# marcinmiklitz/pywindow

Hardware: AMD Instinct MI355X
Metric: trajectory frames/sec full_analysis (pore+windows), CC3 1k-frame (higher is better)
Workload: dtype f64

## Files before the change

pywindow_amd/csrc/pw_kernels.hip:

```cpp
#include <hip/hip_runtime.h>
#include <atomic>
#include <stdio.h>
#include <stdlib.h>
#include <string.h>
#include <time.h>

#include <algorithm>
#include <mutex>
#include <new>

#include "../../include/pywindow_amd.h"
#include "pw_host.hpp"
#include "pw_stat_host.hpp"
#include <vector>
#include "pw_unit.hpp"
#include "pw_launch.hpp"

using namespace pw;

extern "C" int pw_hostpath_run(const pw_batch_in* in, unsigned stages, pw_unit_out* out, const pw_params* prm, int p_cap,
                               int threads, pw_unit_debug* dbg, pw_extra_window* xw, unsigned xw_cap, unsigned* xw_count);
extern "C" int pw_hostpath_default_threads(void);
extern "C" void pw_hostpath_math(int which, const double* x, const double* y, long n, double* out);
extern "C" size_t pw_internal_big_block_bytes(int nmax, int p_cap);
// ... 456 lines not shown
    HostBatch* host;
    long n_units;
    long n_atoms;
    int nmax;
    int vstride;
    unsigned long long* d_ready;
    unsigned long long* h_ready;
    long ready_units;
    int pending;
    unsigned pending_stages;
    long* d_offset;
    double* d_xyz;
    double* d_vdw;
    double* d_mass;
    unsigned char* d_tmpl;
    void* block;
    size_t block_bytes;
    void* parts[5];
    size_t part_bytes[5];
    pw_unit_out* d_out;
    pw_unit_out* d_outs[PW_SETS];
    pw_extra_window* d_xw[PW_SETS];
    unsigned* d_xw_count;
    unsigned xw_cap;
    int nbuf;
    int cur;
    hipEvent_t ev_read[PW_SETS];
    int read_valid[PW_SETS];
    int written_set[PW_SETS];
};

static int block_take(pw_context* c, size_t bytes, void** out, size_t* got) {
    bytes = (bytes + 65535) & ~(size_t)65535;
    int best = -1;
    for (int i = 0; i < (int)c->blocks->size(); ++i) {
        const size_t b = (*c->blocks)[i].bytes;
        if (b >= bytes && b <= 2 * bytes + (1u << 20) && (best < 0 || b < (*c->blocks)[best].bytes)) best = i;
    }
    if (best >= 0) {
        *out = (*c->blocks)[best].p;
        *got = (*c->blocks)[best].bytes;
        c->blocks_bytes -= *got;
        c->blocks->erase(c->blocks->begin() + best);
        return PW_OK;
    }
    HIP_TRY(hipMalloc(out, bytes));
    *got = bytes;
    return PW_OK;
}
static void block_give(pw_context* c, void* p, size_t bytes) {
    if (!p) return;
    if (c && c->blocks && c->blocks->size() < 96 && c->blocks_bytes + bytes <= ((size_t)8 << 30)) {
        c->blocks->push_back({p, bytes});
// ... 98 lines not shown
    if (getenv("PW_PLAN_DEBUG"))
        fprintf(stderr, "launch NW=%d mask %x grid %d lds %zu nmax %d units %ld atoms %ld\n", NW, MASK, p.grid, p.lds,
                r->nmax, r->n_units, r->n_atoms);
    {
        static std::atomic<unsigned long long> done{0};
        unsigned long long bit = 1ull << (c->device & 63);
        if (!(done.load(std::memory_order_acquire) & bit)) {
            HIP_TRY(hipFuncSetAttribute((const void*)kern, hipFuncAttributeMaxDynamicSharedMemorySize,
                                        160 * 1024 - 256 - (int)PW_KERNEL_STATIC_LDS));
            done.fetch_or(bit, std::memory_order_release);
        }
    }
    if (reset_counter) HIP_TRY(hipMemsetAsync(c->counter + counter_slot, 0, sizeof(unsigned long long), st));
    PwWsArgs wsa;
    wsa.ws = c->ws + ws_first;
    wsa.slab = c->slab + (size_t)ws_first * team_slab_bytes(c->p_cap);
    wsa.adj = adj_first >= 0 ? c->adj + (size_t)adj_first * team_adj_words(c->p_cap) : (unsigned long long*)nullptr;
    wsa.xwin = r->d_xw[r->cur];
    wsa.xwin_count = r->d_xw_count + r->cur;
    wsa.xwin_cap = r->xw_cap;
    wsa.p_cap = c->p_cap;
    wsa.nb_off = c->nb_off; wsa.nb_idx = c->nb_idx; wsa.nb_bound = c->nb_bound; wsa.nb_unit = c->nb_unit;
    wsa.wait_ticks = c->wait_ticks * (1 + r->nmax / 512); wsa.stream_wait_ticks = c->stream_wait_ticks;
    hipLaunchKernelGGL(kern, dim3(p.grid), dim3(NW * 64), p.lds, st, r->n_units, r->d_offset,
                       r->d_xyz, r->d_vdw, r->d_mass, stages, r->nmax, p.nrot, p.nlb, p.nframes, p.lean, wsa,
                       c->counter + counter_slot, r->d_out, role, c->cur_queue, c->cur_slots, c->prm, c->rsq_tab,
                       r->vstride, (const unsigned long long*)r->d_ready, (const unsigned char*)r->d_tmpl);
    HIP_TRY(hipGetLastError());
    return PW_OK;
}
static int launch_plan(pw_context* c, pw_resident* r, unsigned stages, const LaunchPlan& p, hipStream_t st,
                       int ws_first, int adj_first, int counter_slot, int role = PW_ROLE_PLAIN,
                       bool reset_counter = true) {
    if (stages == MASK_CHAINS && p.nw == 1)
        return launch_nw<1, MASK_CHAINS>(c, r, stages, p, st, ws_first, adj_first, counter_slot, role, reset_counter);
    if (stages == MASK_WINDOWS && p.nw == 4)
        return launch_nw<4, MASK_WINDOWS>(c, r, stages, p, st, ws_first, adj_first, counter_slot, role, reset_counter);
    if (stages == MASK_WINDOWS_AVG && p.nw == 4)
        return launch_nw<4, MASK_WINDOWS_AVG>(c, r, stages, p, st, ws_first, adj_first, counter_slot, role, reset_counter);
    if (p.nw == 1 && (stages & ~MASK_CHAINS) == 0)
        return launch_nw<1, MASK_CHAINS>(c, r, stages, p, st, ws_first, adj_first, counter_slot, role, reset_counter);
    if (p.nw != 4) {
        snprintf(g_err, sizeof(g_err), "internal: no kernel for %d-wave teams with stages 0x%x", p.nw, stages);
        return PW_E_BAD_ARG;
    }
    return launch_nw<4, MASK_ANY>(c, r, stages, p, st, ws_first, adj_first, counter_slot, role, reset_counter);
// ... 451 lines not shown
                HIP_TRY(hipDeviceSynchronize());
                if (c->bigmem) HIP_TRY(hipFree(c->bigmem));
                c->bigmem = nullptr;
                c->bigmem_bytes = 0;
                HIP_TRY(hipMalloc((void**)&c->bigmem, bb * (size_t)grid));
                c->bigmem_bytes = bb * (size_t)grid;
            }
            c->need_fork = 1;
            rc = join_pipeline(c);
            if (rc != PW_OK) return rc;
            if (r->read_valid[r->cur]) {
                HIP_TRY(hipStreamWaitEvent(c->stream, r->ev_read[r->cur], 0));
                r->read_valid[r->cur] = 0;
            }
            r->written_set[r->cur] = -1;
            HIP_TRY(hipMemsetAsync(r->d_xw_count + r->cur, 0, sizeof(unsigned), c->stream));
            HIP_TRY(hipMemsetAsync(c->counter + 4 * PW_SETS + 1, 0, sizeof(unsigned long long), c->stream));
            PwWsArgs wsa;
            wsa.ws = c->ws; wsa.slab = c->slab; wsa.adj = c->adj;
            wsa.xwin = r->d_xw[r->cur]; wsa.xwin_count = r->d_xw_count + r->cur; wsa.xwin_cap = r->xw_cap;
            wsa.p_cap = c->p_cap;
            wsa.nb_off = c->nb_off; wsa.nb_idx = c->nb_idx; wsa.nb_bound = c->nb_bound; wsa.nb_unit = c->nb_unit;
            wsa.wait_ticks = c->wait_ticks; wsa.stream_wait_ticks = c->stream_wait_ticks;
            return pw_internal_big_launch((void*)c->stream, (int)grid, r->n_units, r->d_offset, r->d_xyz, r->d_vdw, r->d_mass,
                                          stages, r->nmax, &wsa, c->bigmem, bb, c->counter + 4 * PW_SETS + 1, r->d_out, &c->prm,
                                          c->rsq_tab, r->vstride);
        }
    }
    const bool large = wanted_p_cap(c) > PW_P_CAP_PIPELINE;
    const bool pipeline = !c->fused && (stages & PW_STAGE_WINDOWS) != 0 && !large;
    if (!pipeline) {
        LaunchPlan p;
        bool win = (stages & PW_STAGE_WINDOWS) != 0;
        bool opt = win || (stages & PW_STAGE_OPT);
        rc = plan_launch(c, r->n_units, r->nmax, (win || (stages & PW_STAGE_AVG)) ? 4 : 1, win,
                         win ? -1 : (opt ? 1 : 0), &p);
        if (rc != PW_OK) return rc;
        if (large) {
            const size_t per = team_ws_bytes(wanted_p_cap(c), win);
            const size_t budget = (size_t)48 << 30;
            if (per > ((size_t)192 << 30)) {
                snprintf(g_err, sizeof(g_err), "%d sampling vectors per molecule need %zu GB of workspace per team",
                         wanted_p_cap(c), per >> 30);
                return PW_E_TOO_LARGE;
            }
            long g = (long)(budget / per);
// ... 216 lines not shown
            if (n <= 0) snprintf(g_err, sizeof(g_err), "unit %ld has %ld atoms", u, n);
            else snprintf(g_err, sizeof(g_err), "unit %ld has %ld atoms, the template %ld", u, n, (long)in->template_atoms);
            return PW_E_BAD_ARG;
        }
        if (n > nmax) nmax = (int)n;
    }
    r->nmax = nmax;
    r->vstride = in->template_atoms > 0 ? 0 : 1;
    const long nconst = in->template_atoms > 0 ? (long)in->template_atoms : natoms;
#define UP_TRY(call)                          \
    do {                                      \
        hipError_t e_ = (call);               \
        if (e_ != hipSuccess) {               \
            set_err(#call, e_);               \
            pw_resident_free(c, r);           \
            return PW_E_HIP;                  \
        }                                     \
    } while (0)
    if (r->n_units) {
        r->nbuf = c->nsets ? c->nsets : auto_sets(r->n_units);
        auto up256 = [](size_t b) { return (b + 255) & ~(size_t)255; };
        const size_t b_off = up256(sizeof(long) * (size_t)(r->n_units + 1)), b_xyz = up256(sizeof(double) * 3 * (size_t)natoms);
        const size_t b_con = up256(sizeof(double) * (size_t)nconst);
        const size_t b_out = up256((size_t)r->nbuf * sizeof(pw_unit_out) * (size_t)r->n_units + 64);
        const size_t b_tmpl = in->template_atoms > 0 ? up256(template_groups_bytes(nmax)) : 0;
        {
            int rcb = block_take(c, b_off + b_xyz + 2 * b_con + b_tmpl + b_out, &r->block, &r->block_bytes);
            if (rcb != PW_OK) { pw_resident_free(c, r); return rcb; }
        }
        unsigned char* base = (unsigned char*)r->block;
        r->d_offset = (long*)base; base += b_off;
        r->d_xyz = (double*)base; base += b_xyz;
        r->d_vdw = (double*)base; base += b_con;
        r->d_mass = (double*)base; base += b_con;
        std::vector<unsigned char> tmpl_host;
        if (b_tmpl) {
            r->d_tmpl = base; base += b_tmpl;
            tmpl_host.resize(template_groups_bytes(nmax));
            template_groups_build(in->vdw, in->mass, nmax, tmpl_host.data());
        }
        r->d_outs[0] = (pw_unit_out*)base;
        for (int k = 1; k < r->nbuf; ++k) r->d_outs[k] = r->d_outs[0] + (size_t)k * r->n_units;
        r->d_xw_count = (unsigned*)(r->d_outs[0] + (size_t)r->nbuf * r->n_units);
        for (int k = 0; k < PW_SETS; ++k) r->written_set[k] = -1;
        r->d_out = r->d_outs[0];
        r->cur = 0;
        UP_TRY(hipMemcpyAsync(r->d_offset, in->atom_offset, sizeof(long) * (r->n_units + 1),
                              hipMemcpyHostToDevice, c->stream));
        UP_TRY(hipMemcpyAsync(r->d_xyz, in->xyz, sizeof(double) * 3 * natoms, hipMemcpyHostToDevice,
                              c->stream));
        UP_TRY(hipMemcpyAsync(r->d_vdw, in->vdw, sizeof(double) * nconst, hipMemcpyHostToDevice,
                              c->stream));
        UP_TRY(hipMemcpyAsync(r->d_mass, in->mass, sizeof(double) * nconst, hipMemcpyHostToDevice,
                              c->stream));
        if (r->d_tmpl) UP_TRY(hipMemcpyAsync(r->d_tmpl, tmpl_host.data(), tmpl_host.size(), hipMemcpyHostToDevice, c->stream));
        UP_TRY(hipMemsetAsync(r->d_outs[0], 0, r->nbuf * sizeof(pw_unit_out) * r->n_units + 64, c->stream));
        UP_TRY(hipStreamSynchronize(c->stream));
    }
#undef UP_TRY
    c->need_fork = 1;
    *out = r;
    return PW_OK;
}

int pw_resident_stream_begin(pw_context* c, int64_t n_units, int64_t template_atoms, const double* vdw, const double* mass,
                             pw_resident** out) {
    if (!c || !out || n_units <= 0 || template_atoms <= 0 || !vdw || !mass) return PW_E_BAD_ARG;
    PW_LOCK_CONTEXT(c);
    *out = nullptr;
    PW_HOST_UNSUPPORTED(c, "streamed batches");
    if (template_atoms > 40000 || n_units * template_atoms > (int64_t)1 << 40) return PW_E_TOO_LARGE;
    {
        const int pcap = wanted_p_cap(c) > c->p_cap ? wanted_p_cap(c) : c->p_cap;
        if (UnitShared::bytes((int)template_atoms, 1, 1, 1, false, pcap) + 64 > 160 * 1024 - 256 - PW_KERNEL_STATIC_LDS) {
            snprintf(g_err, sizeof(g_err), "molecule with %ld atoms: beyond LDS, upload it in one piece", (long)template_atoms);
            return PW_E_TOO_LARGE;
        }
    }
    PW_ON_DEVICE(c->device);
    pw_resident* r = new (std::nothrow) pw_resident();
    if (!r) return PW_E_NOMEM;
    memset((void*)r, 0, sizeof(*r));
    r->n_units = (long)n_units;
    r->n_atoms = (long)(n_units * template_atoms);
    r->nmax = (int)template_atoms;
    r->vstride = 0;
    r->nbuf = c->nsets ? c->nsets : auto_sets(r->n_units);
    auto up256 = [](size_t b) { return (b + 255) & ~(size_t)255; };
    const size_t b_off = up256(sizeof(long) * (size_t)(r->n_units + 1)), b_xyz = up256(sizeof(double) * 3 * (size_t)r->n_atoms);
    const size_t b_con = up256(sizeof(double) * (size_t)template_atoms);
    const size_t b_out = up256((size_t)r->nbuf * sizeof(pw_unit_out) * (size_t)r->n_units + 64);
    const size_t b_tmpl = up256(template_groups_bytes((int)template_atoms));
    int rcb = block_take(c, b_off + b_xyz + 2 * b_con + b_tmpl + b_out + 256, &r->block, &r->block_bytes);
    if (rcb != PW_OK) { pw_resident_free(c, r); return rcb; }
    unsigned char* base = (unsigned char*)r->block;
    r->d_offset = (long*)base; base += b_off;
    r->d_xyz = (double*)base; base += b_xyz;
    r->d_vdw = (double*)base; base += b_con;
    r->d_mass = (double*)base; base += b_con;
    r->d_tmpl = base; base += b_tmpl;
    std::vector<unsigned char> tmpl_host(template_groups_bytes((int)template_atoms));
    template_groups_build(vdw, mass, (int)template_atoms, tmpl_host.data());
    r->d_outs[0] = (pw_unit_out*)base; base += b_out;
    {
        constexpr unsigned RING = 4096;
        if (!c->ready_vals) {
            hipError_t eh = hipHostMalloc((void**)&c->ready_vals, RING * sizeof(unsigned long long), hipHostMallocMapped | hipHostMallocCoherent);
            if (eh == hipSuccess) eh = hipHostGetDevicePointer((void**)&c->ready_dev, c->ready_vals, 0);
            if (eh != hipSuccess) { set_err("pw_resident_stream_begin (ready counters)", eh); c->ready_vals = nullptr; pw_resident_free(c, r); return PW_E_HIP; }
        }
        const unsigned at = c->ready_at++ % RING;
        r->h_ready = c->ready_vals + at;
        r->d_ready = c->ready_dev + at;
        __atomic_store_n(r->h_ready, 0ull, __ATOMIC_RELEASE);
    }
    for (int k = 1; k < r->nbuf; ++k) r->d_outs[k] = r->d_outs[0] + (size_t)k * r->n_units;
    r->d_xw_count = (unsigned*)(r->d_outs[0] + (size_t)r->nbuf * r->n_units);
    for (int k = 0; k < PW_SETS; ++k) r->written_set[k] = -1;
    r->d_out = r->d_outs[0];
    std::vector<long> off((size_t)r->n_units + 1);
    for (long u = 0; u <= r->n_units; ++u) off[(size_t)u] = u * (long)template_atoms;
    hipError_t e = hipMemcpyAsync(r->d_offset, off.data(), sizeof(long) * (r->n_units + 1), hipMemcpyHostToDevice, c->stream);
    if (e == hipSuccess) e = hipMemcpyAsync(r->d_vdw, vdw, sizeof(double) * template_atoms, hipMemcpyHostToDevice, c->stream);
    if (e == hipSuccess) e = hipMemcpyAsync(r->d_mass, mass, sizeof(double) * template_atoms, hipMemcpyHostToDevice, c->stream);
    if (e == hipSuccess) e = hipMemcpyAsync(r->d_tmpl, tmpl_host.data(), tmpl_host.size(), hipMemcpyHostToDevice, c->stream);
    if (e == hipSuccess) e = hipMemsetAsync(r->d_outs[0], 0, r->nbuf * sizeof(pw_unit_out) * r->n_units + 64, c->stream);
    if (e == hipSuccess) e = hipStreamSynchronize(c->stream);
    if (e != hipSuccess) { set_err("pw_resident_stream_begin", e); pw_resident_free(c, r); return PW_E_HIP; }
    c->need_fork = 1;
    *out = r;
    return PW_OK;
}

int pw_resident_stream_append(pw_context* c, pw_resident* r, const double* xyz, int64_t first, int64_t count) {
    if (!c || !r || !xyz || count < 0) return PW_E_BAD_ARG;
    PW_LOCK_CONTEXT(c);
    if (!r->d_ready || first != r->ready_units || first + count > r->n_units) {
        snprintf(g_err, sizeof(g_err), "pw_resident_stream_append: units %ld..%ld do not continue the %ld appended so far (of %ld)",
                 (long)first, (long)(first + count), r->ready_units, r->n_units);
        return PW_E_BAD_ARG;
    }
    if (count == 0) return PW_OK;
    PW_ON_DEVICE(c->device);
    const size_t per = (size_t)r->nmax * 3;
    HIP_TRY(hipMemcpyAsync(r->d_xyz + (size_t)first * per, xyz, sizeof(double) * per * (size_t)count, hipMemcpyHostToDevice, c->stream));
    HIP_TRY(hipStreamSynchronize(c->stream));
    r->ready_units = (long)(first + count);
    __atomic_store_n(r->h_ready, (unsigned long long)r->ready_units, __ATOMIC_RELEASE);
    if (r->pending && r->ready_units == r->n_units) return pw_resident_launch(c, r, r->pending_stages);
    return PW_OK;
}

int pw_internal_resident_adopt(pw_context* c, long n_units, long n_atoms, int nmax, long* d_offset, double* d_xyz,
                               double* d_vdw, double* d_mass, const size_t* part_bytes, pw_resident** out) {
    if (!c || !out || n_units <= 0 || nmax <= 0 || !part_bytes) return PW_E_BAD_ARG;
    PW_LOCK_CONTEXT(c);
    PW_HOST_UNSUPPORTED(c, "device batches");
    PW_ON_DEVICE(c->device);
    pw_resident* r = new (std::nothrow) pw_resident();
    if (!r) return PW_E_NOMEM;
    memset((void*)r, 0, sizeof(*r));
    r->nbuf = c->nsets ? c->nsets : auto_sets(n_units);
    void* outs = nullptr;
    size_t outs_bytes = 0;
    int rcb = block_take(c, r->nbuf * sizeof(pw_unit_out) * (size_t)n_units + 64, &outs, &outs_bytes);
    if (rcb != PW_OK) { delete r; return rcb; }
    r->d_outs[0] = (pw_unit_out*)outs;
    hipError_t e = hipMemsetAsync(r->d_outs[0], 0, r->nbuf * sizeof(pw_unit_out) * n_units + 64, c->stream);
    if (e == hipSuccess) e = hipStreamSynchronize(c->stream);
    if (e != hipSuccess) {
        set_err("pw_internal_resident_adopt", e);
        block_give(c, outs, outs_bytes);
        delete r;
        return PW_E_HIP;
    }
    r->n_units = n_units; r->n_atoms = n_atoms; r->nmax = nmax; r->vstride = 1;
    r->d_offset = d_offset; r->d_xyz = d_xyz; r->d_vdw = d_vdw; r->d_mass = d_mass;
    r->parts[0] = d_offset; r->parts[1] = d_xyz; r->parts[2] = d_vdw; r->parts[3] = d_mass; r->parts[4] = outs;
    for (int k = 0; k < 4; ++k) r->part_bytes[k] = part_bytes[k];
    r->part_bytes[4] = outs_bytes;
    for (int k = 1; k < r->nbuf; ++k) r->d_outs[k] = r->d_outs[0] + (size_t)k * n_units;
    r->d_xw_count = (unsigned*)(r->d_outs[0] + (size_t)r->nbuf * n_units);
    for (int k = 0; k < PW_SETS; ++k) r->written_set[k] = -1;
    r->d_out = r->d_outs[0];
    r->cur = 0;
    c->need_fork = 1;
    *out = r;
    return PW_OK;
}

static int fetch_extra_windows(pw_context* c, pw_resident* r, unsigned count) {
    c->extra->clear();
    if (count == 0) return PW_OK;
    if (count > r->xw_cap) {
        HIP_TRY(hipDeviceSynchronize());
        if (r->d_xw[0]) HIP_TRY(hipFree(r->d_xw[0]));
        for (int k = 0; k < PW_SETS; ++k) r->d_xw[k] = nullptr;
        r->xw_cap = 0;
        const unsigned cap = ((count + count / 2 + 1023u) / 1024u) * 1024u;
        HIP_TRY(hipMalloc((void**)&r->d_xw[0], (size_t)r->nbuf * cap * sizeof(pw_extra_window)));
        for (int k = 1; k < r->nbuf; ++k) r->d_xw[k] = r->d_xw[0] + (size_t)k * cap;
        r->xw_cap = cap;
        snprintf(g_err, sizeof(g_err), "%u windows beyond the %d a record holds: launch the analysis again "
                 "(the list for them has been allocated)", count, PW_W_MAX);
        return PW_E_RETRY;
// ... 511 lines not shown
```

pywindow_amd/csrc/pw_launch.hpp:

```cpp
#pragma once
#include "../../include/pywindow_amd.h"

struct PwWsArgs {
    void* ws;
    unsigned char* slab;
    unsigned long long* adj;
    pw_extra_window* xwin;
    unsigned* xwin_count;
    unsigned xwin_cap;
    int p_cap;
    const unsigned* nb_off;
    const unsigned short* nb_idx;
    const double* nb_bound;
    const double* nb_unit;
    long long wait_ticks;
    long long stream_wait_ticks;
};

struct UnitQueue {
    unsigned long long tail;
    unsigned long long head;
    int error;
    int started;
};
enum : int { PW_ROLE_PLAIN = 0, PW_ROLE_PRODUCER = 1, PW_ROLE_CONSUMER = 2 };

#if defined(__HIPCC__)
template <class WS>
__device__ inline void bind_workspace(WS* ws, const PwWsArgs& a, unsigned team, const unsigned* rsq_tab, size_t slab_bytes,
                                      size_t adj_words) {
    bind_team_slab(ws, a.slab + (size_t)team * slab_bytes, a.p_cap);
    ws->adj = a.adj ? a.adj + (size_t)team * adj_words : nullptr;
    ws->xwin = a.xwin; ws->xwin_count = a.xwin_count; ws->xwin_cap = a.xwin_cap;
    ws->nb_off = a.nb_off; ws->nb_idx = a.nb_idx; ws->nb_bound = a.nb_bound; ws->nb_unit = a.nb_unit;
    ws->rsq = rsq_tab;
}
#endif
```

pywindow_amd/csrc/pw_unit.hpp:

```cpp
#pragma once
#include "../../include/pywindow_amd.h"
#include "pw_lbfgsb.hpp"
#include "pw_math.hpp"
#include "pw_team.hpp"
#include <string.h>

#if defined(PW_PROFILE) && defined(__HIPCC__)
__shared__ unsigned long long pw_prof_lds[32];
#define PW_PROF_BASE(ws) ((unsigned long long*)pw_prof_lds)
#endif
#if defined(PW_PROFILE) && defined(__HIP_DEVICE_COMPILE__)
#define PW_T0(var) long long var = wall_clock64()
#if defined(PW_ZPROF) && defined(PW_LB_FINE)
#define PW_T1(ws, slot, var) do { (void)var; } while (0)
#elif defined(PW_BARRIER_PROF)
#define PW_T1(ws, slot, var) do { (void)var; if (T::lane() == 0) { unsigned long long w_ = 0; \
        for (int k_ = 0; k_ < T::NWAVES; ++k_) w_ += atomicExch(&pw_bar_acc[k_], 0ull); \
        atomicAdd(&pw_prof_lds[slot], w_); } } while (0)
#else
#define PW_T1(ws, slot, var) do { if (T::lane() == 0) atomicAdd(&pw_prof_lds[slot], (unsigned long long)(wall_clock64() - var)); } while (0)
#endif
#else
#define PW_T0(var) do {} while (0)
#define PW_T1(ws, slot, var) do {} while (0)
// ... 29 lines not shown
    double* pts;
    double* vals;
    int* surv_k;
    int* labels;
    unsigned char* flag;
    unsigned long long* adj;
    double* xw;
    int* xw_ok;
    int p_cap;
    const unsigned* nb_off;
    const unsigned short* nb_idx;
    const double* nb_unit;
    const double* nb_bound;
    pw_extra_window* xwin;
    unsigned* xwin_count;
    unsigned xwin_cap;
    double leaf[256];
    double acc8[8 * 160];
    int leaf_tab[324];
    unsigned long long prof[32];
    const unsigned* rsq;
    pw_unit_debug* dbg_base;
    long unit;
};
PW_HD inline size_t team_slab_bytes(int p_cap) { return (size_t)p_cap * 192; }
PW_HD inline size_t team_adj_words(int p_cap) { return (size_t)p_cap * (size_t)(p_cap / 64); }
PW_HD inline int round_p_cap(long p) {
    if (p < PW_P_MAX) p = PW_P_MAX;
    return (int)((p + 127) & ~127l);
}
PW_HD inline int params_p_cap(double adjust_windows, double adjust_average) {
    double a = adjust_windows > adjust_average ? adjust_windows : adjust_average;
    if (!(a > 0.0)) a = 1.0;
    double want = 2100.0 * a;
    if (want > 4.0e6) want = 4.0e6;
    return round_p_cap((long)want + 1);
}
PW_HD inline void bind_team_slab(TeamWorkspace* ws, unsigned char* slab, int p_cap) {
    const size_t p = (size_t)p_cap;
    double* d = (double*)slab;
    ws->knn = d; d += 10 * p;
    ws->pts = d; d += 3 * p;
    ws->vals = d; d += p;
    ws->xw = d; d += 7 * p;
    int* i = (int*)d;
    ws->surv_k = i; i += p;
// ... 9 lines not shown
    int mw_given;
    double centroid[3];
    double maxd;
    int maxd_i, maxd_j;
    double pore_g;
    int pore_atom;
    double opt_c[3];
    double opt_g;
    int opt_atom;
    double shift[3];
    ClassInfo cls;
    int cls_cnt[PW_KCLS];
    double eps;
    double radius;
    int P;
    int n_surv;
    int n_clusters;
    int n_eval;
    int status;
    double red_v[16];
    int red_i[16];
    int md_list[64];
    int md_count;
    int win_first;
    double win_vec[PW_W_MAX][3];
    int win_ok[PW_W_MAX];
    double win_d[PW_W_MAX];
    double win_c[PW_W_MAX][3];
};

struct UnitShared {
    PW_LDS UnitVars* v;
    ldouble* vdw;
    ldouble* mass;
    lint* perm;
    lint* inv;
    Frame A;
    Frame S;
    Frame R[8];
    PW_LDS void* lb[8];
    PW_LDS unsigned long long* bits[3];
    size_t rot_words;
    int nslots;
    PW_LDS unsigned char* scratch;
    size_t scratch_bytes;
    PW_HD static size_t bytes(int nmax, int nrot, int nlb, int nframes = 2, int lean = 0, int pcap = PW_P_MAX) {
// ... 1682 lines not shown
    }
    PW_HD explicit GramEdgeRule(int n) {
        t0 = applies(n) ? 8 * (n / 8) : 0x40000000;
        panel = last_panel_start(n);
        panel_wide = 12 * (panel / 12);
        nfull = 32 * (n / 32);
        limlast = 12 * ((n - nfull) / 12);
    }
    PW_HD bool is_edge(int o) const { return (unsigned)(o - t0) < 4u; }
    PW_HD bool in_wide_kernel(int o) const {
        return o < panel ? o < panel_wide : (o & 31) < (o < nfull ? 24 : limlast);
    }
    PW_HD bool pair_uses_edge_order(int oi, int oj) const {
        return (is_edge(oi) && in_wide_kernel(oj)) || (is_edge(oj) && in_wide_kernel(oi));
    }
};
template <bool EDGE>
PW_HD inline __attribute__((always_inline)) double pw_gram_nn(double xi, double yi, double zi, double xj, double yj,
                                                              double zj, int oi, int oj, const GramEdgeRule& er) {
    if (EDGE && er.pair_uses_edge_order(oi, oj)) return pw_fma(zi, zj, xi * xj + yi * yj);
    return pw_fma(zi, zj, pw_fma(yi, yj, xi * xj));
}

#if defined(__HIP_DEVICE_COMPILE__)
template <class T, bool VALUE_ONLY, bool EDGE>
__device__ inline __attribute__((always_inline)) bool team_max_dim_few(UnitShared& sh, const Frame& F, int n,
                                                                       const GramEdgeRule& er, const double* centre) {
    auto& v = *sh.v;
    const double cx = centre ? centre[0] : 0.0, cy = centre ? centre[1] : 0.0, cz = centre ? centre[2] : 0.0;
    double smax = -PW_INF, nmax = 0.0;
    int imax = 0x7fffffff;
    for (int i = T::tid(); i < n; i += T::SIZE) {
        const double dx = F.x[i] - cx, dy = F.y[i] - cy, dz = F.z[i] - cz;
        const double si = pw_sqrt(dx * dx + dy * dy + dz * dz) + F.vdw[i];
        if (si > smax) { smax = si; imax = i; }
        nmax = pw_max(nmax, F.xx[i]);
    }
    T::wave_argmax(smax, imax);
    nmax = -T::wave_min(-nmax);
    if (T::lane() == 0) { v.red_v[T::wave()] = smax; v.red_i[T::wave()] = imax; v.red_v[8 + T::wave()] = nmax; }
    T::sync();
    {
        double bb = v.red_v[0], nn = v.red_v[8];
        int bi = v.red_i[0];
        for (int w = 1; w < T::NWAVES; ++w) {
            if (v.red_v[w] > bb || (v.red_v[w] == bb && v.red_i[w] < bi)) { bb = v.red_v[w]; bi = v.red_i[w]; }
            nn = pw_max(nn, v.red_v[8 + w]);
        }
        smax = bb; imax = bi; nmax = nn;
    }
// ... 1 lines not shown
    if (!(smax < PW_INF) || imax >= n) return false;
    const double xi = F.x[imax], yi = F.y[imax], zi = F.z[imax], xxi = F.xx[imax], vi = F.vdw[imax];
    const int oi = F.perm[imax];
    double L = -PW_INF;
    for (int j = T::tid(); j < n; j += T::SIZE) {
        const int oj = F.perm[j];
        double d = 0.0;
        if (j != imax) {
            const double gg = pw_gram_nn<EDGE>(xi, yi, zi, F.x[j], F.y[j], F.z[j], oi, oj, er);
            const double d2 = (oi < oj) ? pw_m2add(gg, xxi) + F.xx[j] : pw_m2add(gg, F.xx[j]) + xxi;
            d = pw_sqrt(d2 > 0.0 ? d2 : 0.0);
        }
        L = pw_max(L, d + (vi + F.vdw[j]));
    }
    L = -T::wave_min(-L);
    if (T::lane() == 0) v.red_v[T::wave()] = L;
    T::sync();
    L = v.red_v[0];
    for (int w = 1; w < T::NWAVES; ++w) L = pw_max(L, v.red_v[w]);
    T::sync();
    if (!(L < PW_INF)) return false;
    const double margin = 1e-6 + 4e-15 * nmax / pw_max(L, 1e-3);
    const double thr = (L - smax) - margin;
    if (T::tid() == 0) v.md_count = 0;
    T::sync();
    for (int i0 = 0; i0 < n; i0 += T::SIZE) {
        const int i = i0 + T::tid();
        bool in = false;
        if (i < n) {
            const double dx = F.x[i] - cx, dy = F.y[i] - cy, dz = F.z[i] - cz;
            in = pw_sqrt(dx * dx + dy * dy + dz * dz) + F.vdw[i] >= thr;
        }
        const unsigned long long mk = T::ballot(in);
        int base = 0;
        if (T::lane() == 0 && mk) base = atomicAdd((PW_LDS int*)&v.md_count, (int)__builtin_popcountll(mk));
        base = __builtin_amdgcn_readfirstlane(base);
        const int at = base + (int)__builtin_popcountll(mk & ((1ull << T::lane()) - 1ull));
        if (in && at < 64) v.md_list[at] = i;
    }
    T::sync();
    const int m = v.md_count;
    if (m > 64) { T::sync(); return false; }
    double bv = -PW_INF, bidx = PW_INF;
    for (int p = T::tid(); p < m * m; p += T::SIZE) {
        const int a = p / m, b = p - a * m;
        const int ia = v.md_list[a], ib = v.md_list[b];
        const int oa = F.perm[ia], ob = F.perm[ib];
        if (oa > ob) continue;
        double d = 0.0;
        if (ia != ib) {
            const double gg = pw_gram_nn<EDGE>(F.x[ia], F.y[ia], F.z[ia], F.x[ib], F.y[ib], F.z[ib], oa, ob, er);
            const double d2 = pw_m2add(gg, F.xx[ia]) + F.xx[ib];
            d = pw_sqrt(d2 > 0.0 ? d2 : 0.0);
        }
        const double val = d + (F.vdw[ia] + F.vdw[ib]);
        const double idx = (double)(oa * n + ob);
        if (val > bv || (val == bv && idx < bidx)) { bv = val; bidx = idx; }
    }
    int ii = (int)(bidx < 2147483647.0 ? bidx : 2147483647.0);
    T::wave_argmax(bv, ii);
    if (T::lane() == 0) { v.red_v[T::wave()] = bv; v.red_i[T::wave()] = ii; }
    T::sync();
    if (T::tid() == 0) {
        double bb = v.red_v[0];
        int bi = v.red_i[0];
        for (int w = 1; w < T::NWAVES; ++w) {
            const double vv = v.red_v[w];
            const int vi2 = v.red_i[w];
            if (vv > bb || (vv == bb && vi2 < bi)) { bb = vv; bi = vi2; }
        }
        v.maxd = bb;
        if (!VALUE_ONLY) { v.maxd_i = bi / n; v.maxd_j = bi % n; }
    }
    T::sync();
    return true;
}
#endif

template <class T, bool VALUE_ONLY = false, bool EDGE = false>
PW_HD inline __attribute__((always_inline)) void team_max_dim_body(UnitShared& sh, const Frame& F, int n,
                                                                   double* item_best = nullptr, const double* centre = nullptr) {
    const GramEdgeRule er(n);
#if defined(__HIP_DEVICE_COMPILE__)
    if (T::WSIZE == 64 && team_max_dim_few<T, VALUE_ONLY, EDGE>(sh, F, n, er, centre)) return;
#else
    (void)centre;
#endif
    const auto& C = *F.cls;
    const int ngrp = C.k;
    const int R = (n + 1) / 2;
    int K = 1;
    {
        long best_cost = 0x7fffffffffffffffl;
        for (int k = 1; k <= 4; ++k) {
            long passes = ((long)R * k + T::SIZE - 1) / T::SIZE;
            long cost = passes * ((n - 1 + 64 / k + k - 1) / k);
            if (cost < best_cost) { best_cost = cost; K = k; }
        }
    }
    const int nitem = R * K;
    double best = -PW_INF;
    if (ngrp > 0) {
        for (int t = T::tid(); t < nitem; t += T::SIZE) {
            const int p = t / K, q = t - p * K;
            double ibest = -PW_INF;
            for (int side = 0; side < 2; ++side) {
                const int i = side == 0 ? p : n - 1 - p;
                if (side == 1 && i == p) break;
                const double xi = F.x[i], yi = F.y[i], zi = F.z[i], xxi = F.xx[i], vi = F.vdw[i];
                const int oi = F.perm[i];
// ... 141 lines not shown
        for (int w = 1; w < T::NWAVES; ++w) bi = pw_min(bi, sh.v->red_v[w]);
        int idx = (int)bi;
        sh.v->maxd = vmax;
        sh.v->maxd_i = idx / n;
        sh.v->maxd_j = idx % n;
    }
    T::sync();
}

template <class T, bool VALUE_ONLY = false>
PW_HD inline __attribute__((always_inline)) void team_max_dim_impl(UnitShared& sh, const Frame& F, int n,
                                                                   double* item_best = nullptr, const double* centre = nullptr) {
    if (GramEdgeRule::applies(n)) team_max_dim_body<T, VALUE_ONLY, true>(sh, F, n, item_best, centre);
    else team_max_dim_body<T, VALUE_ONLY, false>(sh, F, n, item_best, centre);
}

template <class T, bool VALUE_ONLY = false>
PW_NOINLINE PW_HD inline void team_max_dim(UnitShared& sh, const Frame& F, int n, double* item_best = nullptr,
                                           const double* centre = nullptr) {
    team_max_dim_impl<T, VALUE_ONLY>(sh, F, n, item_best, centre);
}

template <class T>
PW_HD inline __attribute__((always_inline)) void stage_basic_impl(UnitShared& sh, TeamWorkspace* ws, int n,
                                                                  pw_unit_out* out, bool com_only) {
    auto& v = *sh.v;
    (void)ws;
    ldouble* cols = seq_sum_columns<T>(sh, n);
    if (cols) {
        const size_t np = (size_t)((n + 1) & ~1);
        for (int i = T::tid(); i < n; i += T::SIZE) {
            const int pos = sh.inv[i];
            const double m = sh.mass[i];
            cols[i] = sh.A.x[pos] * m; cols[np + i] = sh.A.y[pos] * m; cols[2 * np + i] = sh.A.z[pos] * m;
        }
    }
    if (T::tid() == 0 && !v.mw_given) v.mw = molecular_weight_sum((const double*)sh.mass, n);
    T::sync();
    if (cols) {
        seq_sum_columns_add<T>(cols, n, [&](int c, double s) { v.com[c] = s / v.mw; });
    } else {
    auto com_comp = [&](int c) {
        const ldouble* a = c == 0 ? sh.A.x : (c == 1 ? sh.A.y : sh.A.z);
        double s = seq_sum_blocked(n, [&](int i) { return a[sh.inv[i]] * sh.mass[i]; });
        v.com[c] = s / v.mw;
    };
// ... 199 lines not shown
            out->opt_msg = bad ? 0 : S->msg;
        }
    }
    T::sync();
}

template <class T>
PW_NOINLINE PW_HD inline void stage_opt(UnitShared& sh, TeamWorkspace* ws, int n, pw_unit_out* out,
                                        const pw_params& prm) {
    stage_opt_impl<T>(sh, ws, n, out, prm);
}

template <class T>
PW_NOINLINE PW_HD inline void stage_average(UnitShared& sh, TeamWorkspace* ws, int n, pw_unit_out* out,
                                             const pw_params& prm) {
    auto& v = *sh.v;
    PW_T0(t_a0);
    make_shifted<T>(sh, n, v.com[0], v.com[1], v.com[2]);
    double keep_d = v.maxd;
    int keep_i = v.maxd_i, keep_j = v.maxd_j;
    T::sync();
    {
        double* ib = 2 * n + 2 <= ws->p_cap ? ws->vals : nullptr;
        team_max_dim<T, true>(sh, sh.S, n, ib);
    }
    double radius = v.maxd;
    T::sync();
    if (T::tid() == 0) { v.maxd = keep_d; v.maxd_i = keep_i; v.maxd_j = keep_j; }
    int P = sampling_count(radius, prm.adjust_average);
    if (P > ws->p_cap) {
        if (T::tid() == 0) { v.status |= PW_ST_POINTS_OVERFLOW; out->avg_d = __builtin_nan(""); out->n_points_avg = P; }
        T::sync();
        return;
    }
    Sphere sp;
    sp.init(radius, P);
    ScratchArena arena;
    arena.init(sh);
    double* vals = (double*)arena.take((size_t)P * 8);
    if (!vals) vals = ws->vals;
    double* packed = vals;
    unsigned char* flag = (unsigned char*)arena.take((size_t)P);
    if (!flag) flag = ws->flag;
    int* s_tab = (int*)arena.take(324 * 4);
    size_t acc_words = 8 * (size_t)(((P < 8192 ? P : 8192) + 63) / 64);
    if (acc_words < 128) acc_words = 128;
    double* s_acc = (double*)arena.take(acc_words * 8);
// ... 817 lines not shown
            for (int q = 0; q < 10; ++q) rows[(size_t)(k0 + p) * 10 + q] = pw_sqrt(t[p][q]);
        }
}

template <class T>
PW_HD inline __attribute__((always_inline)) int windows_bulk_impl(UnitShared& sh, TeamWorkspace* ws, int n, pw_unit_out* out,
                                                                  const pw_params& prm, WinArrays& wa) {
    auto& v = *sh.v;
    if (T::tid() == 0) {
        for (int c = 0; c < 3; ++c) {
            double adjust = prm.pore_opt ? v.com[c] - v.opt_c[c] : 0.0;
            v.shift[c] = v.com[c] - adjust;
        }
        for (int w = 0; w < 8; ++w) v.red_i[8 + w] = 0;
    }
    T::sync();
    PW_T0(t_pre);
    make_shifted<T>(sh, n, v.shift[0], v.shift[1], v.shift[2]);
    double keep_d = v.maxd;
    int keep_i = v.maxd_i, keep_j = v.maxd_j;
    T::sync();
    if (T::wave() == 0) PW_T1(ws, 14, t_pre);
    PW_T0(t_md);
    team_max_dim<T, true>(sh, sh.S, n, 2 * n + 2 <= ws->p_cap ? ws->vals : nullptr);
    double radius = v.maxd / 2.0;
    T::sync();
    if (T::wave() == 0) PW_T1(ws, 15, t_md);
    if (T::tid() == 0) { v.maxd = keep_d; v.maxd_i = keep_i; v.maxd_j = keep_j; }
    if (!(radius / prm.increment < PW_PATH_POINTS_MAX) || !(radius / prm.increment2 < PW_PATH_POINTS_MAX)) {
        if (T::tid() == 0) {
            v.status |= PW_ST_PATH_TOO_LONG;
            out->n_points = 0; out->sphere_r = radius; out->n_windows = -1; out->n_clusters = 0; out->n_survivors = 0; out->eps = 0.0;
        }
        T::sync();
        return -1;
    }
    int P = sampling_count(radius, prm.adjust_windows);
    if (T::tid() == 0) {
        out->n_points = P;
        out->sphere_r = radius;
        out->n_windows = -1;
        out->n_clusters = 0;
        out->n_survivors = 0;
        out->eps = 0.0;
    }
    if (P > ws->p_cap || P < 10) {
        if (T::tid() == 0) v.status |= P < 10 ? PW_ST_TOO_FEW_POINTS : PW_ST_POINTS_OVERFLOW;
// ... 486 lines not shown
}

template <class T>
PW_NOINLINE PW_HD inline void stage_windows(UnitShared& sh, TeamWorkspace* ws, int n, pw_unit_out* out,
                                             const pw_params& prm) {
    stage_windows_impl<T>(sh, ws, n, out, prm);
}

constexpr unsigned PW_STAGE_REUSE_OPT = 16u;
constexpr unsigned PW_STAGE_MERGE = 32u;
constexpr unsigned PW_STAGE_COM_ONLY = 64u;

PW_HD inline void record_or_status(pw_unit_out* out, int st, int evals) {
#if defined(__HIP_DEVICE_COMPILE__)
    if (st) atomicOr(&out->status, st);
    atomicAdd(&out->n_eval, evals);
#else
    out->status |= st;
    out->n_eval += evals;
#endif
}

template <class T>
PW_HD inline void analyse_unit(UnitShared& sh, TeamWorkspace* ws, int n, const double* xyz,
                               const double* vdw, const double* mass, unsigned stages,
                               pw_unit_out* out, const pw_params& prm, const unsigned char* tmpl = nullptr) {
    const bool merge = (stages & PW_STAGE_MERGE) != 0;
    const bool reuse_opt = (stages & PW_STAGE_REUSE_OPT) != 0;
    if ((stages & PW_STAGE_WINDOWS) && !reuse_opt && prm.pore_opt) stages |= PW_STAGE_OPT;
    if (T::tid() == 0 && !merge) {
        out->status = 0;
        out->n_eval = 0;
        out->avg_d = 0.0;
        out->pore_opt_d = 0.0; out->pore_opt_atom = -1; out->pore_vol_opt = 0.0;
        out->pore_opt_c[0] = out->pore_opt_c[1] = out->pore_opt_c[2] = 0.0;
        out->n_windows = -1; out->n_clusters = 0;
        out->n_points = 0; out->n_points_avg = 0; out->n_survivors = 0;
        out->opt_nit = 0; out->opt_nfev = 0; out->opt_task = 0; out->opt_msg = 0;
        out->eps = 0.0; out->sphere_r = 0.0;
        for (int w = 0; w < PW_W_MAX; ++w) {
            out->win_d[w] = 0.0;
            out->win_c[w][0] = out->win_c[w][1] = out->win_c[w][2] = 0.0;
        }
    }
    PW_T0(t_load);
    load_unit<T>(sh, n, xyz, vdw, mass, tmpl);
    if (T::wave() == 0) PW_T1(ws, 5, t_load);
    if (reuse_opt) {
        if (T::tid() == 0) { sh.v->com[0] = out->com[0]; sh.v->com[1] = out->com[1]; sh.v->com[2] = out->com[2]; }
        T::sync();
    } else {
        stage_basic<T>(sh, ws, n, out, (stages & PW_STAGE_COM_ONLY) != 0);
    }
    if (stages & PW_STAGE_OPT) stage_opt<T>(sh, ws, n, out, prm);
    if (reuse_opt) {
        if (T::tid() == 0) {
            sh.v->opt_c[0] = out->pore_opt_c[0];
            sh.v->opt_c[1] = out->pore_opt_c[1];
            sh.v->opt_c[2] = out->pore_opt_c[2];
            if (out->status & PW_ST_NEGATIVE_PORE) sh.v->status |= PW_ST_NEGATIVE_PORE;
        }
        T::sync();
    }
    if (stages & PW_STAGE_AVG) {
        PW_T0(t_a);
        stage_average<T>(sh, ws, n, out, prm);
        if (T::wave() == 0) PW_T1(ws, 13, t_a);
        if ((stages & PW_STAGE_WINDOWS) && sh.S.x == sh.A.x) {
            for (int i = T::tid(); i < n; i += T::SIZE) {
                const int pos = sh.inv[i];
                const double x = xyz[3 * i], y = xyz[3 * i + 1], z = xyz[3 * i + 2];
                sh.A.x[pos] = x; sh.A.y[pos] = y; sh.A.z[pos] = z;
                sh.A.xx[pos] = sq3(x, y, z);
            }
            T::sync();
        }
    }
    if (stages & PW_STAGE_WINDOWS) {
        if (!(prm.pore_opt && (sh.v->status & PW_ST_NEGATIVE_PORE))) {
            stage_windows<T>(sh, ws, n, out, prm);
        }
        else if (T::tid() == 0) out->n_windows = -1;
    }
    if (T::tid() == 0) {
        if (merge) {
            record_or_status(out, sh.v->status, sh.v->n_eval);
        } else {
            out->status = sh.v->status;
            out->n_eval = sh.v->n_eval;
        }
    }
    T::sync();
}

}
```

Before: 1.064 million.

## Carry max-dimension candidate atom list across stages and pipeline kernels

Records the small candidate atom list from the max-dimension search in basic stage, along with L and nmax, and reuses it for the later shifted max-dim calls in the windows and pore stages. An error bound decides when the reuse is safe. The list is also handed between pipeline roles through a new side buffer placed after the per-unit output records, so the reuse-opt kernel can skip rebuilding it. The goal is to avoid repeated O(n) list builds and full max-dim fallbacks, at the cost of extra per-unit global memory and added control flow. Host-path compilation of the few-candidate path is also enabled.

```diff
diff --git a/pywindow_amd/csrc/pw_kernels.hip b/pywindow_amd/csrc/pw_kernels.hip
--- a/pywindow_amd/csrc/pw_kernels.hip
+++ b/pywindow_amd/csrc/pw_kernels.hip
@@ -502,6 +502,7 @@
     pw_unit_out* d_outs[PW_SETS];
     pw_extra_window* d_xw[PW_SETS];
     unsigned* d_xw_count;
+    unsigned char* d_md;
     unsigned xw_cap;
     int nbuf;
     int cur;
@@ -509,6 +510,10 @@
     int read_valid[PW_SETS];
     int written_set[PW_SETS];
 };
+
+static size_t records_bytes(int nbuf, long n_units) { return ((size_t)nbuf * sizeof(pw_unit_out) * (size_t)n_units + 64 + 255) & ~(size_t)255; }
+static size_t result_area_bytes(int nbuf, long n_units) { return records_bytes(nbuf, n_units) + (size_t)nbuf * (size_t)n_units * PW_MD_SIDE_STRIDE; }
+static unsigned char* md_side_of(pw_unit_out* outs, int nbuf, long n_units) { return (unsigned char*)outs + records_bytes(nbuf, n_units); }
 
 static int block_take(pw_context* c, size_t bytes, void** out, size_t* got) {
     bytes = (bytes + 65535) & ~(size_t)65535;
@@ -653,6 +658,7 @@
     wsa.p_cap = c->p_cap;
     wsa.nb_off = c->nb_off; wsa.nb_idx = c->nb_idx; wsa.nb_bound = c->nb_bound; wsa.nb_unit = c->nb_unit;
     wsa.wait_ticks = c->wait_ticks * (1 + r->nmax / 512); wsa.stream_wait_ticks = c->stream_wait_ticks;
+    wsa.md_side = role != PW_ROLE_PLAIN && r->d_md ? r->d_md + (size_t)r->cur * (size_t)r->n_units * PW_MD_SIDE_STRIDE : nullptr;
     hipLaunchKernelGGL(kern, dim3(p.grid), dim3(NW * 64), p.lds, st, r->n_units, r->d_offset,
                        r->d_xyz, r->d_vdw, r->d_mass, stages, r->nmax, p.nrot, p.nlb, p.nframes, p.lean, wsa,
                        c->counter + counter_slot, r->d_out, role, c->cur_queue, c->cur_slots, c->prm, c->rsq_tab,
@@ -1150,6 +1156,7 @@
             wsa.p_cap = c->p_cap;
             wsa.nb_off = c->nb_off; wsa.nb_idx = c->nb_idx; wsa.nb_bound = c->nb_bound; wsa.nb_unit = c->nb_unit;
             wsa.wait_ticks = c->wait_ticks; wsa.stream_wait_ticks = c->stream_wait_ticks;
+            wsa.md_side = nullptr;
             return pw_internal_big_launch((void*)c->stream, (int)grid, r->n_units, r->d_offset, r->d_xyz, r->d_vdw, r->d_mass,
                                           stages, r->nmax, &wsa, c->bigmem, bb, c->counter + 4 * PW_SETS + 1, r->d_out, &c->prm,
                                           c->rsq_tab, r->vstride);
@@ -1412,7 +1419,7 @@
         auto up256 = [](size_t b) { return (b + 255) & ~(size_t)255; };
         const size_t b_off = up256(sizeof(long) * (size_t)(r->n_units + 1)), b_xyz = up256(sizeof(double) * 3 * (size_t)natoms);
         const size_t b_con = up256(sizeof(double) * (size_t)nconst);
-        const size_t b_out = up256((size_t)r->nbuf * sizeof(pw_unit_out) * (size_t)r->n_units + 64);
+        const size_t b_out = up256(result_area_bytes(r->nbuf, r->n_units));
         const size_t b_tmpl = in->template_atoms > 0 ? up256(template_groups_bytes(nmax)) : 0;
         {
             int rcb = block_take(c, b_off + b_xyz + 2 * b_con + b_tmpl + b_out, &r->block, &r->block_bytes);
@@ -1432,6 +1439,7 @@
         r->d_outs[0] = (pw_unit_out*)base;
         for (int k = 1; k < r->nbuf; ++k) r->d_outs[k] = r->d_outs[0] + (size_t)k * r->n_units;
         r->d_xw_count = (unsigned*)(r->d_outs[0] + (size_t)r->nbuf * r->n_units);
+        r->d_md = md_side_of(r->d_outs[0], r->nbuf, r->n_units);
         for (int k = 0; k < PW_SETS; ++k) r->written_set[k] = -1;
         r->d_out = r->d_outs[0];
         r->cur = 0;
@@ -1444,7 +1452,7 @@
         UP_TRY(hipMemcpyAsync(r->d_mass, in->mass, sizeof(double) * nconst, hipMemcpyHostToDevice,
                               c->stream));
         if (r->d_tmpl) UP_TRY(hipMemcpyAsync(r->d_tmpl, tmpl_host.data(), tmpl_host.size(), hipMemcpyHostToDevice, c->stream));
-        UP_TRY(hipMemsetAsync(r->d_outs[0], 0, r->nbuf * sizeof(pw_unit_out) * r->n_units + 64, c->stream));
+        UP_TRY(hipMemsetAsync(r->d_outs[0], 0, result_area_bytes(r->nbuf, r->n_units), c->stream));
         UP_TRY(hipStreamSynchronize(c->stream));
     }
 #undef UP_TRY
@@ -1479,7 +1487,7 @@
     auto up256 = [](size_t b) { return (b + 255) & ~(size_t)255; };
     const size_t b_off = up256(sizeof(long) * (size_t)(r->n_units + 1)), b_xyz = up256(sizeof(double) * 3 * (size_t)r->n_atoms);
     const size_t b_con = up256(sizeof(double) * (size_t)template_atoms);
-    const size_t b_out = up256((size_t)r->nbuf * sizeof(pw_unit_out) * (size_t)r->n_units + 64);
+    const size_t b_out = up256(result_area_bytes(r->nbuf, r->n_units));
     const size_t b_tmpl = up256(template_groups_bytes((int)template_atoms));
     int rcb = block_take(c, b_off + b_xyz + 2 * b_con + b_tmpl + b_out + 256, &r->block, &r->block_bytes);
     if (rcb != PW_OK) { pw_resident_free(c, r); return rcb; }
@@ -1506,6 +1514,7 @@
     }
     for (int k = 1; k < r->nbuf; ++k) r->d_outs[k] = r->d_outs[0] + (size_t)k * r->n_units;
     r->d_xw_count = (unsigned*)(r->d_outs[0] + (size_t)r->nbuf * r->n_units);
+    r->d_md = md_side_of(r->d_outs[0], r->nbuf, r->n_units);
     for (int k = 0; k < PW_SETS; ++k) r->written_set[k] = -1;
     r->d_out = r->d_outs[0];
     std::vector<long> off((size_t)r->n_units + 1);
@@ -1514,7 +1523,7 @@
     if (e == hipSuccess) e = hipMemcpyAsync(r->d_vdw, vdw, sizeof(double) * template_atoms, hipMemcpyHostToDevice, c->stream);
     if (e == hipSuccess) e = hipMemcpyAsync(r->d_mass, mass, sizeof(double) * template_atoms, hipMemcpyHostToDevice, c->stream);
     if (e == hipSuccess) e = hipMemcpyAsync(r->d_tmpl, tmpl_host.data(), tmpl_host.size(), hipMemcpyHostToDevice, c->stream);
-    if (e == hipSuccess) e = hipMemsetAsync(r->d_outs[0], 0, r->nbuf * sizeof(pw_unit_out) * r->n_units + 64, c->stream);
+    if (e == hipSuccess) e = hipMemsetAsync(r->d_outs[0], 0, result_area_bytes(r->nbuf, r->n_units), c->stream);
     if (e == hipSuccess) e = hipStreamSynchronize(c->stream);
     if (e != hipSuccess) { set_err("pw_resident_stream_begin", e); pw_resident_free(c, r); return PW_E_HIP; }
     c->need_fork = 1;
@@ -1553,10 +1562,10 @@
     r->nbuf = c->nsets ? c->nsets : auto_sets(n_units);
     void* outs = nullptr;
     size_t outs_bytes = 0;
-    int rcb = block_take(c, r->nbuf * sizeof(pw_unit_out) * (size_t)n_units + 64, &outs, &outs_bytes);
+    int rcb = block_take(c, result_area_bytes(r->nbuf, n_units), &outs, &outs_bytes);
     if (rcb != PW_OK) { delete r; return rcb; }
     r->d_outs[0] = (pw_unit_out*)outs;
-    hipError_t e = hipMemsetAsync(r->d_outs[0], 0, r->nbuf * sizeof(pw_unit_out) * n_units + 64, c->stream);
+    hipError_t e = hipMemsetAsync(r->d_outs[0], 0, result_area_bytes(r->nbuf, n_units), c->stream);
     if (e == hipSuccess) e = hipStreamSynchronize(c->stream);
     if (e != hipSuccess) {
         set_err("pw_internal_resident_adopt", e);
@@ -1571,6 +1580,7 @@
     r->part_bytes[4] = outs_bytes;
     for (int k = 1; k < r->nbuf; ++k) r->d_outs[k] = r->d_outs[0] + (size_t)k * n_units;
     r->d_xw_count = (unsigned*)(r->d_outs[0] + (size_t)r->nbuf * n_units);
+    r->d_md = md_side_of(r->d_outs[0], r->nbuf, n_units);
     for (int k = 0; k < PW_SETS; ++k) r->written_set[k] = -1;
     r->d_out = r->d_outs[0];
     r->cur = 0;
diff --git a/pywindow_amd/csrc/pw_launch.hpp b/pywindow_amd/csrc/pw_launch.hpp
--- a/pywindow_amd/csrc/pw_launch.hpp
+++ b/pywindow_amd/csrc/pw_launch.hpp
@@ -15,6 +15,7 @@
     const double* nb_unit;
     long long wait_ticks;
     long long stream_wait_ticks;
+    unsigned char* md_side;
 };
 
 struct UnitQueue {
@@ -34,5 +35,6 @@
     ws->xwin = a.xwin; ws->xwin_count = a.xwin_count; ws->xwin_cap = a.xwin_cap;
     ws->nb_off = a.nb_off; ws->nb_idx = a.nb_idx; ws->nb_bound = a.nb_bound; ws->nb_unit = a.nb_unit;
     ws->rsq = rsq_tab;
+    ws->md_side = a.md_side;
 }
 #endif
diff --git a/pywindow_amd/csrc/pw_unit.hpp b/pywindow_amd/csrc/pw_unit.hpp
--- a/pywindow_amd/csrc/pw_unit.hpp
+++ b/pywindow_amd/csrc/pw_unit.hpp
@@ -75,6 +75,7 @@
     const unsigned* rsq;
     pw_unit_debug* dbg_base;
     long unit;
+    unsigned char* md_side;
 };
 PW_HD inline size_t team_slab_bytes(int p_cap) { return (size_t)p_cap * 192; }
 PW_HD inline size_t team_adj_words(int p_cap) { return (size_t)p_cap * (size_t)(p_cap / 64); }
@@ -130,6 +131,8 @@
     int red_i[16];
     int md_list[64];
     int md_count;
+    int md_valid;
+    double md_L, md_nmax;
     int win_first;
     double win_vec[PW_W_MAX][3];
     int win_ok[PW_W_MAX];
@@ -1858,10 +1861,9 @@
     return pw_fma(zi, zj, pw_fma(yi, yj, xi * xj));
 }
 
-#if defined(__HIP_DEVICE_COMPILE__)
-template <class T, bool VALUE_ONLY, bool EDGE>
-__device__ inline __attribute__((always_inline)) bool team_max_dim_few(UnitShared& sh, const Frame& F, int n,
-                                                                       const GramEdgeRule& er, const double* centre) {
+template <class T, bool EDGE>
+PW_HD inline __attribute__((always_inline)) bool team_max_dim_list_build(UnitShared& sh, const Frame& F, int n,
+                                                                         const GramEdgeRule& er, const double* centre) {
     auto& v = *sh.v;
     const double cx = centre ? centre[0] : 0.0, cy = centre ? centre[1] : 0.0, cz = centre ? centre[2] : 0.0;
     double smax = -PW_INF, nmax = 0.0;
@@ -1909,7 +1911,7 @@
     if (!(L < PW_INF)) return false;
     const double margin = 1e-6 + 4e-15 * nmax / pw_max(L, 1e-3);
     const double thr = (L - smax) - margin;
-    if (T::tid() == 0) v.md_count = 0;
+    if (T::tid() == 0) { v.md_count = 0; v.md_L = L; v.md_nmax = nmax; }
     T::sync();
     for (int i0 = 0; i0 < n; i0 += T::SIZE) {
         const int i = i0 + T::tid();
@@ -1920,14 +1922,25 @@
         }
         const unsigned long long mk = T::ballot(in);
         int base = 0;
+#if defined(__HIP_DEVICE_COMPILE__)
         if (T::lane() == 0 && mk) base = atomicAdd((PW_LDS int*)&v.md_count, (int)__builtin_popcountll(mk));
         base = __builtin_amdgcn_readfirstlane(base);
+#else
+        base = v.md_count;
+        v.md_count += (int)__builtin_popcountll(mk);
+#endif
         const int at = base + (int)__builtin_popcountll(mk & ((1ull << T::lane()) - 1ull));
         if (in && at < 64) v.md_list[at] = i;
     }
     T::sync();
     const int m = v.md_count;
     if (m > 64) { T::sync(); return false; }
+    return true;
+}
+template <class T, bool VALUE_ONLY, bool EDGE>
+PW_HD inline __attribute__((always_inline)) void team_max_dim_list_eval(UnitShared& sh, const Frame& F, int n,
+                                                                        const GramEdgeRule& er, int m) {
+    auto& v = *sh.v;
     double bv = -PW_INF, bidx = PW_INF;
     for (int p = T::tid(); p < m * m; p += T::SIZE) {
         const int a = p / m, b = p - a * m;
@@ -1960,19 +1973,50 @@
         if (!VALUE_ONLY) { v.maxd_i = bi / n; v.maxd_j = bi % n; }
     }
     T::sync();
+}
+template <class T, bool VALUE_ONLY, bool EDGE>
+PW_HD inline __attribute__((always_inline)) bool team_max_dim_few(UnitShared& sh, const Frame& F, int n,
+                                                                  const GramEdgeRule& er, const double* centre) {
+    auto& v = *sh.v;
+    if (T::tid() == 0) v.md_valid = 0;
+    if (!team_max_dim_list_build<T, EDGE>(sh, F, n, er, centre)) return false;
+    const int m = v.md_count;
+    if (!VALUE_ONLY && T::tid() == 0) v.md_valid = 1;
+    team_max_dim_list_eval<T, VALUE_ONLY, EDGE>(sh, F, n, er, m);
     return true;
 }
-#endif
+
+constexpr double MAXDIM_CARRY_LIMIT = 1e-9;
+PW_HD inline bool max_dim_list_carries(double L, double nmax_a, double shift_sq) {
+    const double r = pw_sqrt(nmax_a) + pw_sqrt(shift_sq);
+    const double e = 4e-15 * (nmax_a + 2.0 * (r * r)) / pw_max(L, 1e-3);
+    return e < MAXDIM_CARRY_LIMIT;
+}
+template <class T>
+PW_HD inline __attribute__((always_inline)) bool team_max_dim_carried(UnitShared& sh, const Frame& F, int n, const double* shift) {
+#ifdef PW_NO_MAXDIM_LIST
+    (void)sh; (void)F; (void)n; (void)shift;
+    return false;
+#else
+    auto& v = *sh.v;
+    if (!v.md_valid) return false;
+    const int m = v.md_count;
+    if (m < 1 || m > 64 || !max_dim_list_carries(v.md_L, v.md_nmax, sq3(shift[0], shift[1], shift[2]))) return false;
+    const GramEdgeRule er(n);
+    if (GramEdgeRule::applies(n)) team_max_dim_list_eval<T, true, true>(sh, F, n, er, m);
+    else team_max_dim_list_eval<T, true, false>(sh, F, n, er, m);
+    return true;
+#endif
+}
+constexpr int PW_MD_SIDE_STRIDE = 64 * 2 + 8 + 8 + 8;
+struct MdSideEntry { unsigned short list[64]; int count; int pad; double L, nmax; };
+static_assert(sizeof(MdSideEntry) == PW_MD_SIDE_STRIDE, "max_dim list hand-over entry");
 
 template <class T, bool VALUE_ONLY = false, bool EDGE = false>
 PW_HD inline __attribute__((always_inline)) void team_max_dim_body(UnitShared& sh, const Frame& F, int n,
                                                                    double* item_best = nullptr, const double* centre = nullptr) {
     const GramEdgeRule er(n);
-#if defined(__HIP_DEVICE_COMPILE__)
     if (T::WSIZE == 64 && team_max_dim_few<T, VALUE_ONLY, EDGE>(sh, F, n, er, centre)) return;
-#else
-    (void)centre;
-#endif
     const auto& C = *F.cls;
     const int ngrp = C.k;
     const int R = (n + 1) / 2;
@@ -2160,6 +2204,12 @@
 }
 
 template <class T>
+PW_NOINLINE PW_HD inline void team_max_dim_shifted(UnitShared& sh, const Frame& F, int n, double* item_best, const double* shift) {
+    if (team_max_dim_carried<T>(sh, F, n, shift)) return;
+    team_max_dim_impl<T, true>(sh, F, n, item_best, nullptr);
+}
+
+template <class T>
 PW_HD inline __attribute__((always_inline)) void stage_basic_impl(UnitShared& sh, TeamWorkspace* ws, int n,
                                                                   pw_unit_out* out, bool com_only) {
     auto& v = *sh.v;
@@ -2405,7 +2455,7 @@
     T::sync();
     {
         double* ib = 2 * n + 2 <= ws->p_cap ? ws->vals : nullptr;
-        team_max_dim<T, true>(sh, sh.S, n, ib);
+        team_max_dim_shifted<T>(sh, sh.S, n, ib, (const double*)&v.com[0]);
     }
     double radius = v.maxd;
     T::sync();
@@ -3269,7 +3319,7 @@
     T::sync();
     if (T::wave() == 0) PW_T1(ws, 14, t_pre);
     PW_T0(t_md);
-    team_max_dim<T, true>(sh, sh.S, n, 2 * n + 2 <= ws->p_cap ? ws->vals : nullptr);
+    team_max_dim_shifted<T>(sh, sh.S, n, 2 * n + 2 <= ws->p_cap ? ws->vals : nullptr, (const double*)&v.shift[0]);
     double radius = v.maxd / 2.0;
     T::sync();
     if (T::wave() == 0) PW_T1(ws, 15, t_md);
@@ -3802,6 +3852,31 @@
 }
 
 template <class T>
+PW_NOINLINE PW_HD inline void md_side_load(UnitShared& sh, TeamWorkspace* ws) {
+#ifndef PW_NO_MAXDIM_LIST
+    if (!ws->md_side) return;
+    const MdSideEntry* e = (const MdSideEntry*)ws->md_side + ws->unit;
+    const int m = e->count;
+    if (T::tid() < 64 && T::tid() < m) sh.v->md_list[T::tid()] = (int)e->list[T::tid()];
+    if (T::tid() == 0 && m >= 1 && m <= 64) { sh.v->md_count = m; sh.v->md_L = e->L; sh.v->md_nmax = e->nmax; sh.v->md_valid = 1; }
+#else
+    (void)sh; (void)ws;
+#endif
+}
+template <class T>
+PW_NOINLINE PW_HD inline void md_side_store(UnitShared& sh, TeamWorkspace* ws) {
+#ifndef PW_NO_MAXDIM_LIST
+    if (!ws->md_side || T::tid() >= 64) return;
+    MdSideEntry* e = (MdSideEntry*)ws->md_side + ws->unit;
+    const int m = sh.v->md_valid ? sh.v->md_count : 0;
+    if (T::tid() < m) e->list[T::tid()] = (unsigned short)sh.v->md_list[T::tid()];
+    if (T::tid() == 0) { e->count = m; e->L = sh.v->md_L; e->nmax = sh.v->md_nmax; }
+#else
+    (void)sh; (void)ws;
+#endif
+}
+
+template <class T>
 PW_HD inline void analyse_unit(UnitShared& sh, TeamWorkspace* ws, int n, const double* xyz,
                                const double* vdw, const double* mass, unsigned stages,
                                pw_unit_out* out, const pw_params& prm, const unsigned char* tmpl = nullptr) {
@@ -3823,11 +3898,13 @@
             out->win_c[w][0] = out->win_c[w][1] = out->win_c[w][2] = 0.0;
         }
     }
+    if (T::tid() == 0) sh.v->md_valid = 0;
     PW_T0(t_load);
     load_unit<T>(sh, n, xyz, vdw, mass, tmpl);
     if (T::wave() == 0) PW_T1(ws, 5, t_load);
     if (reuse_opt) {
         if (T::tid() == 0) { sh.v->com[0] = out->com[0]; sh.v->com[1] = out->com[1]; sh.v->com[2] = out->com[2]; }
+        md_side_load<T>(sh, ws);
         T::sync();
     } else {
         stage_basic<T>(sh, ws, n, out, (stages & PW_STAGE_COM_ONLY) != 0);
@@ -3862,6 +3939,7 @@
         }
         else if (T::tid() == 0) out->n_windows = -1;
     }
+    if (!reuse_opt) md_side_store<T>(sh, ws);
     if (T::tid() == 0) {
         if (merge) {
             record_or_status(out, sh.v->status, sh.v->n_eval);
```

Result: no change. 1.072 million, median of 6 (+0.8%).
